# TravisWheelerLab/BATH

Hardware: AMD Instinct MI355X
Metric: DP Gcells/s + residues/s through bathsearch pipeline at 1/2/4/8 MI355X (higher is better)
Workload: dtype u8/i16 integer scores (SSV: exact binary16), f32 Forward

## Files before the change

### bath_amd/csrc/bath_orfs.hip

```cpp
#include <algorithm>
#include <climits>
#include <cstring>

#include "bath_common.hpp"
#include "bath_kernels.hpp"
#include "bath_launch.hpp"

namespace bath {

constexpr int kTileLanes = 32;
constexpr int kTileCodons = 4 * kTileLanes;
constexpr int kTileNt = 12 * kTileLanes;

struct OrfScanTables {
  const uint8_t *aa_full;
  const uint8_t *aa64_fwd;
  const uint8_t *aa64_rev;
  const uint8_t *comp;
};

struct OrfTiles {
  const int4 *desc;
  const int32_t *tile_first;
  int64_t ntiles;
};

struct OrfScanOut {
  uint8_t *aa;
  uint2 *slots;
  int32_t *cnt;
  uint2 *cross;
  int32_t *prefix, *suffix;
  int *hist;
  unsigned long long *n_orfs, *orf_res;
  int cap;
  int count;
};

struct OrfFilter {
  int strands;
  int using_initiators;
  const uint8_t *is_init;
  const uint8_t *comp;
};

__device__ __forceinline__ int orf_bin(int len) { return min(len, kOrfBins - 1); }

__device__ __forceinline__ int half_shfl_up(int v, int d) { return __shfl_up(v, d, kTileLanes); }

template <int CTRL, int ROW_MASK = 0xf>
__device__ __forceinline__ int dpp_or_ident(int v, int ident) { return __builtin_amdgcn_update_dpp(ident, v, CTRL, ROW_MASK, 0xf, false); }
__device__ __forceinline__ int half_excl_max_scan(int v, int ident, bool first_lane_of_half) {
  int x = dpp_or_ident<0x138>(v, ident);
  x = first_lane_of_half ? ident : x;
  x = max(x, dpp_or_ident<0x111>(x, ident));
  x = max(x, dpp_or_ident<0x112>(x, ident));
  x = max(x, dpp_or_ident<0x114>(x, ident));
  x = max(x, dpp_or_ident<0x118>(x, ident));
  x = max(x, dpp_or_ident<0x142, 0xa>(x, ident));
  return x;
}

__global__ __launch_bounds__(256) void orf_tile_kernel(SeqView dna, OrfTiles tiles, OrfScanTables tabs, OrfScanOut out, int minlen) {
  __shared__ int s_hist[kOrfBins];
  __shared__ __attribute__((aligned(16))) uint8_t s_full[5832 + 8];
  __shared__ uint16_t s_fr[64];
  __shared__ uint8_t s_comp[32];
  __shared__ unsigned s_red[2];
  __shared__ int s_cnt[8];
  for (int i = threadIdx.x; i < kOrfBins; i += blockDim.x) s_hist[i] = 0;
  for (int i = threadIdx.x; i < 5832; i += blockDim.x) s_full[i] = tabs.aa_full[i];
  if (threadIdx.x < 64) {
    const unsigned f = tabs.aa64_fwd[threadIdx.x], r = tabs.aa64_rev[threadIdx.x];
    s_fr[threadIdx.x] = (uint16_t)((f | (f == kStop ? 0x80u : 0u)) | ((r | (r == kStop ? 0x80u : 0u)) << 8));
  }
  if (threadIdx.x < 18) s_comp[threadIdx.x] = tabs.comp[threadIdx.x];
  if (threadIdx.x < 2) s_red[threadIdx.x] = 0;
  __syncthreads();
  const int hw = threadIdx.x / kTileLanes;
  const int i = threadIdx.x % kTileLanes;
  const int64_t wave0 = ((int64_t)blockIdx.x * blockDim.x + threadIdx.x) >> 6;
  const int64_t nwaves = ((int64_t)gridDim.x * blockDim.x) >> 6;
  unsigned my_orfs = 0, my_res = 0;
  const int half = (threadIdx.x & 63) / kTileLanes;
  const int4 none = {0, 0, 0, 0};
  auto fetch_desc = [&](int64_t tb) { const int64_t t = tb + half; return t < tiles.ntiles ? tiles.desc[t] : none; };
  auto fetch_data = [&](const int4 &dsc, uint32_t (&D)[4]) {
    const int p0 = kTileNt * dsc.w + 12 * i;
    D[0] = D[1] = D[2] = D[3] = 0u;
    if (p0 < dsc.y) {
      const uint8_t *d = dna.data + ((int64_t)(uint32_t)dsc.x << 4) + p0;
#pragma unroll
      for (int k = 0; k < 4; k++) D[k] = *reinterpret_cast<const uint32_t *>(d + 4 * k);
    }
  };
  const int64_t tstep = nwaves * 2;
  int4 d_next = fetch_desc(wave0 * 2), d_next2 = fetch_desc(wave0 * 2 + tstep);
  uint32_t D_next[4];
  fetch_data(d_next, D_next);
  for (int64_t tb = wave0 * 2; tb < tiles.ntiles; tb += tstep) {
    const int64_t tile = tb + half;
    const int4 dsc = d_next;
    uint32_t D[4] = {D_next[0], D_next[1], D_next[2], D_next[3]};
    d_next = d_next2;
    d_next2 = fetch_desc(tb + 2 * tstep);
    fetch_data(d_next, D_next);
    const int n = dsc.y;
    const bool live = n > 0;
    const int w = dsc.z, T = dsc.w;
    const int64_t off = (int64_t)(uint32_t)dsc.x << 4;
    const int p0 = kTileNt * T + 12 * i;
    if (i == 0) s_cnt[hw] = 0;
#pragma unroll
    for (int k = 0; k < 4; k++) {
      const int rem = n - (p0 + 4 * k);
      if (rem < 4) D[k] = (rem <= 0) ? 0u : (D[k] & ((1u << (8 * rem)) - 1u));
    }
    const bool canonical = ((D[0] | D[1] | D[2] | (D[3] & 0xffffu)) & 0xfcfcfcfcu) == 0u;
    int af[12], ar[12];
    if (__all(canonical)) {
#pragma unroll
      for (int k = 0; k < 12; k++) {
        const unsigned t = (k % 4 == 0) ? D[k / 4] : __builtin_amdgcn_alignbyte(D[k / 4 + 1], D[k / 4], k % 4);
        const unsigned idx = (__umul24(t, 0x100401u) >> 16) & 63u;
        const unsigned e = s_fr[idx];
        af[k] = (int)(e & 0xffu); ar[k] = (int)(e >> 8);
      }
    } else {
#pragma unroll
      for (int k = 0; k < 12; k++) {
        const unsigned t = (k % 4 == 0) ? D[k / 4] : __builtin_amdgcn_alignbyte(D[k / 4 + 1], D[k / 4], k % 4);
        const int x0 = min((int)(t & 0xffu), 17), x1 = min((int)((t >> 8) & 0xffu), 17), x2 = min((int)((t >> 16) & 0xffu), 17);
        const int f = s_full[(x0 * 18 + x1) * 18 + x2];
        const int r = s_full[((int)s_comp[x2] * 18 + (int)s_comp[x1]) * 18 + (int)s_comp[x0]];
        af[k] = f | (f == kStop ? 0x80 : 0); ar[k] = r | (r == kStop ? 0x80 : 0);
      }
    }
    const int nvalid = live ? min(max(n - 2 - p0, 0), 12) : 0;
    const int pitch = orf_stream_pitch(n);
    uint8_t *const abase = out.aa + (2 * off + 96 * (int64_t)w);
    const int u0 = kTileCodons * T + 4 * i;
    unsigned inv[3];
    int cv[3];
#pragma unroll
    for (int ph = 0; ph < 3; ph++) {
      cv[ph] = (max(nvalid - ph + 2, 0) * 11) >> 5;
      inv[ph] = cv[ph] >= 4 ? 0u : (0x80808080u << (8 * cv[ph]));
    }
    const int q3 = n / 3, r3 = n - 3 * q3;
    uint2 *const slots = out.slots + tile * out.cap;
    int *const prefix6 = out.prefix + tile * 6, *const suffix6 = out.suffix + tile * 6;
#pragma unroll
    for (int st = 0; st < 6; st++) {
      const int ph = st % 3;
      const bool rev = st >= 3;
      const int fr = r3 - ph + (r3 < ph ? 3 : 0);
      const int sf = rev ? 3 + fr : ph;
      const int C = q3 - 1 - (r3 < ph ? 1 : 0);
      const int *a = rev ? ar : af;
      const unsigned pk = (unsigned)a[ph] | ((unsigned)a[ph + 3] << 8) | ((unsigned)a[ph + 6] << 16) | ((unsigned)a[ph + 9] << 24);
      const unsigned mf = (pk & 0x80808080u) | inv[ph];
      const int so = sf * pitch + (rev ? C - u0 - 3 : u0);
      if (cv[ph] == 4) {
        *reinterpret_cast<uint32_t *>(abase + so) = rev ? __builtin_amdgcn_perm(0u, pk & 0x7f7f7f7fu, 0x00010203u)  : (pk & 0x7f7f7f7fu);
      } else {
#pragma unroll
        for (int c = 0; c < 4; c++) if (c < cv[ph]) abase[so + (rev ? 3 - c : c)] = (uint8_t)(a[ph + 3 * c] & 0x7f);
      }
      const int mine = mf ? 4 * i + ((31 - (int)__clz(mf)) >> 3) : INT_MIN;
      const int last = half_excl_max_scan(mine, INT_MIN, i == 0);
      bool open = last < 0;
      const int run_in = open ? 4 * i : 4 * i - 1 - last;
      auto record = [&](int u_stop, int len) {
        const int k = atomicAdd(&s_cnt[hw], 1);
        slots[k] = make_uint2((unsigned)(rev ? C - u_stop + 1 : u_stop - len), (unsigned)len | ((unsigned)sf << 28));
        atomicAdd(&s_hist[orf_bin(len)], 1);
        my_orfs++; my_res += (unsigned)len;
      };
      if (minlen > 2) {
        if (mf != 0u) {
          const int first = (__ffs((int)mf) - 1) >> 3;
          const int len = run_in + first;
          if (open) { if (live) prefix6[sf] = len; }
          else if (live && len >= minlen) record(u0 + first, len);
        }
        if (live && i == kTileLanes - 1) {
          suffix6[sf] = mf ? (int)__clz(mf) >> 3 : run_in + 4;
          if (open && mf == 0u) prefix6[sf] = kTileCodons;
        }
      } else {
        int len = run_in;
#pragma unroll
        for (int c = 0; c < 4; c++) {
          if ((mf >> (8 * c + 7)) & 1u) {
            if (open) { if (live) prefix6[sf] = len; open = false; }
            else if (live && len >= minlen) record(u0 + c, len);
            len = 0;
          } else len++;
        }
        if (live && i == kTileLanes - 1) {
          suffix6[sf] = len;
          if (open) prefix6[sf] = kTileCodons;
        }
      }
    }
    if (live && i == 0) out.cnt[tile] = s_cnt[hw];
  }
  if (my_orfs) { atomicAdd(&s_red[0], my_orfs); atomicAdd(&s_red[1], my_res); }
  __syncthreads();
  if (!out.count) return;
  for (int k = threadIdx.x; k < kOrfBins; k += blockDim.x) if (s_hist[k]) atomicAdd(&out.hist[k], s_hist[k]);
  if (threadIdx.x == 0 && s_red[0]) { atomicAdd(out.n_orfs, (unsigned long long)s_red[0]); atomicAdd(out.orf_res, (unsigned long long)s_red[1]); }
}

__global__ __launch_bounds__(256) void orf_stitch_kernel(SeqView dna, OrfTiles tiles, OrfScanOut out, int minlen) {
  __shared__ int s_hist[kOrfBins];
  __shared__ unsigned s_red[2];
  for (int i = threadIdx.x; i < kOrfBins; i += blockDim.x) s_hist[i] = 0;
  if (threadIdx.x < 2) s_red[threadIdx.x] = 0;
  __syncthreads();
  unsigned my_orfs = 0, my_res = 0;
  const int64_t nstreams = dna.n * 6;
  for (int64_t sidx = (int64_t)blockIdx.x * blockDim.x + threadIdx.x; sidx < nstreams; sidx += (int64_t)gridDim.x * blockDim.x) {
    const int64_t w = sidx / 6;
    const int sf = (int)(sidx - w * 6);
    const int n = dna.len[w];
    if (n < 15) continue;
    const int nt = (n / 3) / kTileCodons + 1;
    const int64_t first = tiles.tile_first[w];
    const bool rev = sf >= 3;
    const int fr = rev ? sf - 3 : 0;
    const int ph = rev ? (n - fr) % 3 : sf;
    const int C = (n - 3 - fr - ph) / 3;
    int carry = 0;
    for (int T = 0; T < nt; T++) {
      const int64_t e = (first + T) * 6 + sf;
      const int p = out.prefix[e];
      if (p < kTileCodons) {
        const int len = carry + p;
        uint2 none = make_uint2(0u, 0u);
        if (len < minlen) out.cross[e] = none;
        else {
          const int u_stop = kTileCodons * T + p;
          out.cross[e] = make_uint2((unsigned)(rev ? C - u_stop + 1 : u_stop - len), (unsigned)len | ((unsigned)sf << 28));
          atomicAdd(&s_hist[orf_bin(len)], 1);
          my_orfs++; my_res += (unsigned)len;
        }
        carry = out.suffix[e];
      } else { carry += kTileCodons; out.cross[e] = make_uint2(0u, 0u); }
    }
  }
  if (my_orfs) { atomicAdd(&s_red[0], my_orfs); atomicAdd(&s_red[1], my_res); }
  __syncthreads();
  if (!out.count) return;
  for (int k = threadIdx.x; k < kOrfBins; k += blockDim.x) if (s_hist[k]) atomicAdd(&out.hist[k], s_hist[k]);
  if (threadIdx.x == 0 && s_red[0]) { atomicAdd(out.n_orfs, (unsigned long long)s_red[0]); atomicAdd(out.orf_res, (unsigned long long)s_red[1]); }
}

__device__ __forceinline__ int wave_excl_max_scan(int v, int ident) {
  int x = dpp_or_ident<0x138>(v, ident);
  x = max(x, dpp_or_ident<0x111>(x, ident));
  x = max(x, dpp_or_ident<0x112>(x, ident));
  x = max(x, dpp_or_ident<0x114>(x, ident));
  x = max(x, dpp_or_ident<0x118>(x, ident));
  x = max(x, dpp_or_ident<0x142, 0xa>(x, ident));
  x = max(x, dpp_or_ident<0x143, 0xc>(x, ident));
  return x;
}
__global__ __launch_bounds__(256) void orf_stitch_wave_kernel(SeqView dna, OrfTiles tiles, OrfScanOut out, int minlen) {
  __shared__ int s_hist[kOrfBins];
  __shared__ unsigned s_red[2];
  for (int i = threadIdx.x; i < kOrfBins; i += blockDim.x) s_hist[i] = 0;
  if (threadIdx.x < 2) s_red[threadIdx.x] = 0;
  __syncthreads();
  unsigned my_orfs = 0, my_res = 0;
  const int lane = threadIdx.x & 63;
  const int64_t nstreams = dna.n * 6;
  const int64_t nwaves = ((int64_t)gridDim.x * blockDim.x) >> 6;
  for (int64_t sidx = ((int64_t)blockIdx.x * blockDim.x + threadIdx.x) >> 6; sidx < nstreams; sidx += nwaves) {
    const int64_t w = sidx / 6;
    const int sf = (int)(sidx - w * 6);
    const int n = dna.len[w];
    if (n < 15) continue;
    const int nt = (n / 3) / kTileCodons + 1;
    const int64_t first = tiles.tile_first[w];
    const bool rev = sf >= 3;
    const int fr = rev ? sf - 3 : 0;
    const int ph = rev ? (n - fr) % 3 : sf;
    const int C = (n - 3 - fr - ph) / 3;
    int carry_in = 0;
    for (int T0 = 0; T0 < nt; T0 += 64) {
      const int T = T0 + lane;
      const bool valid = T < nt;
      const int64_t e = (first + (valid ? T : 0)) * 6 + sf;
      const int p = valid ? out.prefix[e] : kTileCodons;
      const bool has = p < kTileCodons;
      const int sfx = has ? out.suffix[e] : 0;
      const int j = wave_excl_max_scan(has ? lane : -1, -1);
      const int sfx_j = __shfl(sfx, j < 0 ? 0 : j, 64);
      const int carry = (j >= 0) ? sfx_j + kTileCodons * (lane - j - 1) : carry_in + kTileCodons * lane;
      if (valid) {
        uint2 rec = make_uint2(0u, 0u);
        if (has) {
          const int len = carry + p;
          if (len >= minlen) {
            const int u_stop = kTileCodons * T + p;
            rec = make_uint2((unsigned)(rev ? C - u_stop + 1 : u_stop - len), (unsigned)len | ((unsigned)sf << 28));
            atomicAdd(&s_hist[orf_bin(len)], 1);
            my_orfs++; my_res += (unsigned)len;
          }
        }
        out.cross[e] = rec;
      }
      const int leave = has ? sfx : carry + kTileCodons;
      carry_in = __shfl(leave, 63, 64);
    }
  }
  if (my_orfs) { atomicAdd(&s_red[0], my_orfs); atomicAdd(&s_red[1], my_res); }
  __syncthreads();
  if (!out.count) return;
  for (int k = threadIdx.x; k < kOrfBins; k += blockDim.x) if (s_hist[k]) atomicAdd(&out.hist[k], s_hist[k]);
  if (threadIdx.x == 0 && s_red[0]) { atomicAdd(out.n_orfs, (unsigned long long)s_red[0]); atomicAdd(out.orf_res, (unsigned long long)s_red[1]); }
}

__global__ __launch_bounds__(256) void orf_filter_kernel(SeqView dna, OrfTiles tiles, OrfScanOut out, OrfFilter flt, int minlen) {
  __shared__ int s_hist[kOrfBins];
  __shared__ unsigned s_red[2];
  __shared__ uint8_t s_init[64], s_comp[32];
  for (int i = threadIdx.x; i < kOrfBins; i += blockDim.x) s_hist[i] = 0;
  if (threadIdx.x < 64) s_init[threadIdx.x] = flt.using_initiators ? flt.is_init[threadIdx.x] : 1;
  if (threadIdx.x < 18) s_comp[threadIdx.x] = flt.comp[threadIdx.x];
  if (threadIdx.x < 2) s_red[threadIdx.x] = 0;
  __syncthreads();
  auto members = [](int x) -> unsigned {
    switch (x) {
      case 0: return 1u; case 1: return 2u; case 2: return 4u; case 3: return 8u;
      case 5: return 5u; case 6: return 10u; case 7: return 3u; case 8: return 12u; case 9: return 6u; case 10: return 9u;
      case 11: return 11u; case 12: return 14u; case 13: return 7u; case 14: return 13u; case 15: return 15u;
      default: return 0u;
    }
  };
  auto initiates = [&](int a, int b, int c) -> bool {
    if ((a | b | c) < 4) return s_init[16 * a + 4 * b + c] != 0;
    const unsigned ma = members(a), mb = members(b), mc = members(c);
    int n = 0;
    for (int x = 0; x < 4; x++) if (ma >> x & 1u)
      for (int y = 0; y < 4; y++) if (mb >> y & 1u)
        for (int z = 0; z < 4; z++) if (mc >> z & 1u) { if (!s_init[16 * x + 4 * y + z]) return false; n++; }
    return n > 0;
  };
  unsigned my_orfs = 0, my_res = 0;
  for (int64_t t = (int64_t)blockIdx.x * blockDim.x + threadIdx.x; t < tiles.ntiles; t += (int64_t)gridDim.x * blockDim.x) {
    const int4 dsc = tiles.desc[t];
    const int n = dsc.y, w = dsc.z;
    if (n < 15) continue;
    const int64_t off = (int64_t)(uint32_t)dsc.x << 4;
    const uint8_t *x = dna.data + off;
    uint8_t *const abase = out.aa + (2 * off + 96 * (int64_t)w);
    const int pitch = orf_stream_pitch(n);
    const int c = out.cnt[t];
    uint2 *sl = out.slots + t * out.cap;
    for (int k = 0; k < c + 6; k++) {
      uint2 *rp = k < c ? sl + k : out.cross + t * 6 + (k - c);
      uint2 r = *rp;
      int len = (int)(r.y & 0x0fffffffu);
      if (len == 0) continue;
      const int sf = (int)(r.y >> 28);
      const bool rev = sf >= 3;
      if ((flt.strands == BATH_STRAND_TOPONLY && rev) || (flt.strands == BATH_STRAND_BOTTOMONLY && !rev)) { rp->y = 0u; continue; }
      if (flt.using_initiators) {
        int j = (int)r.x;
        const int jend = j + len;
        for (; j < jend; j++) {
          int a, b, cc;
          if (!rev) { const int p = sf + 3 * j; a = x[p]; b = x[p + 1]; cc = x[p + 2]; }
          else { const int q = (sf - 3) + 3 * j; a = s_comp[min((int)x[n - 1 - q], 17)]; b = s_comp[min((int)x[n - 2 - q], 17)]; cc = s_comp[min((int)x[n - 3 - q], 17)]; }
          if (initiates(min(a, 17), min(b, 17), min(cc, 17))) break;
        }
        len = jend - j;
        if (len < minlen || len <= 0) { rp->y = 0u; continue; }
        abase[sf * pitch + j] = 10;
        r.x = (unsigned)j; r.y = (unsigned)len | ((unsigned)sf << 28);
        *rp = r;
      }
      atomicAdd(&s_hist[orf_bin(len)], 1);
      my_orfs++; my_res += (unsigned)len;
    }
  }
  if (my_orfs) { atomicAdd(&s_red[0], my_orfs); atomicAdd(&s_red[1], my_res); }
  __syncthreads();
  for (int k = threadIdx.x; k < kOrfBins; k += blockDim.x) if (s_hist[k]) atomicAdd(&out.hist[k], s_hist[k]);
  if (threadIdx.x == 0 && s_red[0]) { atomicAdd(out.n_orfs, (unsigned long long)s_red[0]); atomicAdd(out.orf_res, (unsigned long long)s_red[1]); }
}

__global__ __launch_bounds__(256) void orf_scan_bins(const int *__restrict__ hist, int *__restrict__ cursor, int *__restrict__ n_total) {
  constexpr int kPer = kOrfBins / 256;
  __shared__ int s_wsum[4];
  const int tid = threadIdx.x, lane = tid & 63, wv = tid >> 6;
  int c[kPer], sum = 0;
#pragma unroll
  for (int k = 0; k < kPer; k++) { c[k] = hist[kOrfBins - 1 - (kPer * tid + k)]; sum += c[k]; }
  int x = sum;
#pragma unroll
  for (int d = 1; d < 64; d <<= 1) { const int y = __shfl_up(x, d, 64); if (lane >= d) x += y; }
  if (lane == 63) s_wsum[wv] = x;
  __syncthreads();
  int run = x - sum;
#pragma unroll
  for (int u = 0; u < 4; u++) run += u < wv ? s_wsum[u] : 0;
#pragma unroll
  for (int k = 0; k < kPer; k++) { cursor[(kOrfBins - 1 - (kPer * tid + k)) * kOrfCursorStride] = run; run += c[k]; }
  if (tid == 255) *n_total = run;
}

constexpr int kSortThreads = 1024;
constexpr int kSortTiles = 768;
constexpr int kSortRegs = 16;
constexpr int kSortRound = kSortThreads * kSortRegs;

__global__ __launch_bounds__(kSortThreads) void orf_sort_kernel(OrfTiles tiles, const uint2 *__restrict__ slots, int cap, const int32_t *__restrict__ cnt,
                                                                const uint2 *__restrict__ cross, int *__restrict__ cursor, OrfRec *__restrict__ sorted) {
  __shared__ int s_bin[kOrfBins];
  __shared__ int s_pre[kSortTiles + 1];
  __shared__ int64_t s_wbase[kSortTiles];
  __shared__ int2 s_wp[kSortTiles];
  __shared__ uint16_t s_own[kSortRound];
  __shared__ int s_wsum[kSortThreads / 64];
  const int tid = threadIdx.x, lane = tid & 63, wv = tid >> 6;
  const int64_t t0 = (int64_t)blockIdx.x * kSortTiles;
  int e = 0;
  if (tid < kSortTiles && t0 + tid < tiles.ntiles) {
    const int64_t t = t0 + tid;
    const int4 dsc = tiles.desc[t];
    e = cnt[t] + 6;
    s_wbase[tid] = 2 * ((int64_t)(uint32_t)dsc.x << 4) + 96 * (int64_t)dsc.z;
    s_wp[tid] = make_int2(dsc.z, orf_stream_pitch(dsc.y));
  }
  for (int i = tid; i < kOrfBins; i += kSortThreads) s_bin[i] = 0;
  int x = e;
#pragma unroll
  for (int d = 1; d < 64; d <<= 1) { const int y = __shfl_up(x, d, 64); if (lane >= d) x += y; }
  if (lane == 63) s_wsum[wv] = x;
  __syncthreads();
  int before = 0, total = 0;
#pragma unroll
  for (int u = 0; u < kSortThreads / 64; u++) { const int s = s_wsum[u]; before += u < wv ? s : 0; total += s; }
  const int pre = before + x - e;
  if (tid < kSortTiles) s_pre[tid] = pre;
  if (tid == 0) s_pre[kSortTiles] = total;
  for (int r0 = 0; r0 < total; r0 += kSortRound) {
    if (tid < kSortTiles) {
      const int lo = max(pre, r0) - r0, hi = min(pre + e, r0 + kSortRound) - r0;
      for (int j = lo; j < hi; j++) s_own[j] = (uint16_t)tid;
    }
    __syncthreads();
    uint2 r[kSortRegs];
    int ti[kSortRegs];
#pragma unroll
    for (int k = 0; k < kSortRegs; k++) {
      const int j = r0 + k * kSortThreads + tid;
      r[k] = make_uint2(0u, 0u);
      ti[k] = -1;
      if (j < total) {
        const int i = s_own[j - r0];
        const int loc = j - s_pre[i], c = s_pre[i + 1] - s_pre[i] - 6;
        const int64_t t = t0 + i;
        r[k] = loc < c ? slots[t * cap + loc] : cross[t * 6 + (loc - c)];
        ti[k] = i;
      }
    }
#pragma unroll
    for (int k = 0; k < kSortRegs; k++) {
      const int len = (int)(r[k].y & 0x0fffffffu);
      if (len) ti[k] |= atomicAdd(&s_bin[orf_bin(len)], 1) << 10;
      else ti[k] = -1;
    }
    __syncthreads();
    for (int i = tid; i < kOrfBins; i += kSortThreads) {
      const int c = s_bin[i];
      if (c) s_bin[i] = atomicAdd(&cursor[i * kOrfCursorStride], c);
    }
    __syncthreads();
#pragma unroll
    for (int k = 0; k < kSortRegs; k++) {
      if (ti[k] < 0) continue;
      const int i = ti[k] & 1023, rank = ti[k] >> 10;
      const int2 wp = s_wp[i];
      const int pos = s_bin[orf_bin((int)(r[k].y & 0x0fffffffu))] + rank;
      OrfRec rec;
      rec.aa_off = s_wbase[i] + (int64_t)(r[k].y >> 28) * wp.y + (int64_t)r[k].x; rec.w = wp.x; rec.len_sf = (int32_t)r[k].y;
      sorted[pos] = rec;
    }
    if (r0 + kSortRound < total) {
      __syncthreads();
      for (int i = tid; i < kOrfBins; i += kSortThreads) s_bin[i] = 0;
    }
  }
}

size_t orf_aa_bytes(const bath_hip_seqs *dna) { return (size_t)(2 * dna->total_aligned + 96 * dna->n + 256); }
void orf_buffers_carve(OrfBuffers *ob, void *aa, void *slots, void *sorted, void *misc, size_t nent) {
  ob->aa = static_cast<uint8_t *>(aa); ob->slots = slots; ob->sorted = static_cast<OrfRec *>(sorted);
  ob->cross = misc;
  ob->cnt = static_cast<int32_t *>(misc) + 2 * nent; ob->prefix = ob->cnt + nent; ob->suffix = ob->prefix + nent;
  ob->hist = reinterpret_cast<int *>(ob->suffix + nent); ob->cursor = ob->hist + kOrfBins; ob->ntotal = ob->cursor + kOrfBins * kOrfCursorStride;
}

int orf_slot_cap(int minlen) { return 6 * (kTileCodons / (std::max(minlen, 0) + 1) + 2); }

int orf_tiles_ensure(bath_hip_ctx *ctx, const bath_hip_seqs *dna) {
  if (dna->ntiles >= 0) return BATH_OK;
  std::vector<int32_t> first((size_t)std::max<int64_t>(dna->n, 1));
  std::vector<int4> desc;
  int64_t nt = 0;
  for (int64_t w = 0; w < dna->n; w++) {
    first[(size_t)w] = (int32_t)nt;
    const int n = dna->h_len[(size_t)w];
    const int k = n >= 15 ? (n / 3) / kTileCodons + 1 : 0;
    nt += k;
    if (nt >= (int64_t)INT32_MAX / 8 || (dna->h_off[(size_t)w] >> 4) > (int64_t)UINT32_MAX) { ctx->set_error("DNA block too large for one pipeline call: split it"); return BATH_EINVAL; }
    for (int T = 0; T < k; T++) desc.push_back(int4{(int)(uint32_t)(dna->h_off[(size_t)w] >> 4), n, (int)w, T});
  }
  if (desc.empty()) desc.push_back(int4{0, 0, 0, 0});
  BATH_HIP_TRY(ctx, hipMalloc((void **)&dna->d_tile_desc, desc.size() * sizeof(int4)));
  BATH_HIP_TRY(ctx, hipMalloc((void **)&dna->d_tile_first, first.size() * sizeof(int32_t)));
  BATH_HIP_TRY(ctx, hipMemcpy(dna->d_tile_desc, desc.data(), desc.size() * sizeof(int4), hipMemcpyHostToDevice));
  BATH_HIP_TRY(ctx, hipMemcpy(dna->d_tile_first, first.data(), first.size() * sizeof(int32_t), hipMemcpyHostToDevice));
  dna->ntiles = nt;
  return BATH_OK;
}

static bool dna_degen_has(int x, int y) {
  static const char *members[18] = {"A", "C", "G", "T", "", "AG", "CT", "AC", "GT", "CG", "AT", "ACT", "CGT", "ACG", "AGT", "ACGT", "", ""};
  static const char nt[] = "ACGT";
  return std::strchr(members[x], nt[y]) != nullptr;
}

static void build_codon_table(const uint8_t basic[64], std::vector<uint8_t> &tab) {
  tab.assign(18 * 18 * 18, (uint8_t)kXaa);
  for (int a = 0; a < 18; a++) for (int b = 0; b < 18; b++) for (int c = 0; c < 18; c++) {
    int aa = -1; bool mixed = false;
    for (int x = 0; x < 4 && !mixed; x++) { if (!dna_degen_has(a, x)) continue;
      for (int y = 0; y < 4 && !mixed; y++) { if (!dna_degen_has(b, y)) continue;
        for (int z = 0; z < 4; z++) { if (!dna_degen_has(c, z)) continue;
          int v = basic[16 * x + 4 * y + z];
          if (aa == -1) aa = v; else if (aa != v) { mixed = true; break; }
        } } }
    tab[(a * 18 + b) * 18 + c] = (uint8_t)((mixed || aa == -1) ? kXaa : aa);
  }
}

int orf_tables_upload(bath_hip_ctx *ctx, int ncbi_table, OrfTablesDev *t, int initiator) {
  const int key = ncbi_table | (initiator << 16);
  t->using_initiators = initiator != BATH_INIT_ANY;
  if (ctx->orf_tables_id == key && ctx->scratch[28].p) {
    t->full = ctx->scratch[28].as<uint8_t>(); t->fwd = t->full + 6144; t->rev = t->fwd + 64; t->comp = t->rev + 64; t->is_init = t->comp + 32;
    return BATH_OK;
  }
  uint8_t basic[64];
  if (bath_gencode_basic(ncbi_table, basic) != BATH_OK) { ctx->set_error("unknown NCBI translation table"); return BATH_EINVAL; }
  std::vector<uint8_t> host(6144 + 256, 0);
  std::vector<uint8_t> full;
  build_codon_table(basic, full);
  std::memcpy(host.data(), full.data(), full.size());
  uint8_t *fwd = host.data() + 6144, *rev = fwd + 64, *comp = rev + 64;
  for (int a = 0; a < 4; a++) for (int b = 0; b < 4; b++) for (int c = 0; c < 4; c++) {
    fwd[a * 16 + b * 4 + c] = basic[16 * a + 4 * b + c];
    rev[a * 16 + b * 4 + c] = basic[16 * (3 - c) + 4 * (3 - b) + (3 - a)];
  }
  static const uint8_t kComp[18] = {3, 2, 1, 0, 4, 6, 5, 8, 7, 9, 10, 14, 13, 12, 11, 15, 16, 17};
  std::memcpy(comp, kComp, 18);
  if (bath_gencode_initiators(ncbi_table, initiator, comp + 32) != BATH_OK) { ctx->set_error("no initiation codons for this table / initiator mode"); return BATH_EINVAL; }
  DevBuf &b = ctx->scratch[28];
  BATH_HIP_TRY(ctx, b.reserve(host.size()));
  BATH_HIP_TRY(ctx, hipMemcpyAsync(b.p, host.data(), host.size(), hipMemcpyHostToDevice, ctx->stream));
  BATH_HIP_TRY(ctx, hipStreamSynchronize(ctx->stream));
  ctx->orf_tables_id = key;
  t->full = b.as<uint8_t>(); t->fwd = t->full + 6144; t->rev = t->fwd + 64; t->comp = t->rev + 64; t->is_init = t->comp + 32;
  return BATH_OK;
}

int launch_orf_scan(bath_hip_ctx *ctx, const bath_hip_seqs *dna, const OrfTablesDev &tt, int minlen, const OrfBuffers &b,
                    unsigned long long *d_n_orfs, unsigned long long *d_orf_res, int strands) {
  const int64_t ntiles = dna->ntiles;
  BATH_HIP_TRY(ctx, hipMemsetAsync(b.hist, 0, kOrfBins * sizeof(int), ctx->stream));
  OrfScanTables tabs{tt.full, tt.fwd, tt.rev, tt.comp};
  OrfTiles tiles{reinterpret_cast<const int4 *>(dna->d_tile_desc), dna->d_tile_first, ntiles};
  const bool filtered = strands != BATH_STRAND_BOTH || tt.using_initiators;
  OrfScanOut out{b.aa, reinterpret_cast<uint2 *>(b.slots), b.cnt, reinterpret_cast<uint2 *>(b.cross), b.prefix, b.suffix, b.hist, d_n_orfs, d_orf_res, orf_slot_cap(minlen), filtered ? 0 : 1};
  const int cus = ctx->prop.multiProcessorCount;
  int per_cu = 0;
  if (hipOccupancyMaxActiveBlocksPerMultiprocessor(&per_cu, orf_tile_kernel, 256, 0) != hipSuccess || per_cu < 1) per_cu = 4;
  const int blocks = (int)std::max<int64_t>(1, std::min<int64_t>((ntiles + 7) / 8, (int64_t)cus * per_cu));
  hipLaunchKernelGGL(orf_tile_kernel, dim3(blocks), dim3(256), 0, ctx->stream, dna->view(), tiles, tabs, out, minlen);
  static const int stitch_env = [] { const char *e = std::getenv("BATH_HIP_STITCH_WAVE"); return e ? std::atoi(e) : -1; }();
  const bool long_windows = stitch_env >= 0 ? stitch_env == 1 : ntiles > 32 * dna->n;
  if (long_windows) {
    const int wblocks = (int)std::max<int64_t>(1, std::min<int64_t>((dna->n * 6 + 3) / 4, (int64_t)cus * 8));
    hipLaunchKernelGGL(orf_stitch_wave_kernel, dim3(wblocks), dim3(256), 0, ctx->stream, dna->view(), tiles, out, minlen);
  } else {
  const int sblocks = (int)std::max<int64_t>(1, std::min<int64_t>((dna->n * 6 + 255) / 256, (int64_t)cus * 8));
  hipLaunchKernelGGL(orf_stitch_kernel, dim3(sblocks), dim3(256), 0, ctx->stream, dna->view(), tiles, out, minlen);
  }
  if (filtered) {
    OrfFilter flt{strands, tt.using_initiators ? 1 : 0, tt.is_init, tt.comp};
    const int fblocks = (int)std::max<int64_t>(1, std::min<int64_t>((ntiles + 255) / 256, (int64_t)cus * 8));
    hipLaunchKernelGGL(orf_filter_kernel, dim3(fblocks), dim3(256), 0, ctx->stream, dna->view(), tiles, out, flt, minlen);
  }
  hipLaunchKernelGGL(orf_scan_bins, dim3(1), dim3(256), 0, ctx->stream, b.hist, b.cursor, b.ntotal);
  hipLaunchKernelGGL(orf_sort_kernel, dim3((unsigned)std::max<int64_t>(1, (ntiles + kSortTiles - 1) / kSortTiles)), dim3(kSortThreads), 0, ctx->stream, tiles,
                     reinterpret_cast<const uint2 *>(b.slots), out.cap, b.cnt, reinterpret_cast<const uint2 *>(b.cross), b.cursor, b.sorted);
  BATH_HIP_TRY(ctx, hipGetLastError());
  return BATH_OK;
}

}

using namespace bath;

extern "C" int bath_hip_translate_orfs(bath_hip_ctx *ctx, const bath_hip_seqs *dna, int ncbi_table, int min_orf_len,
                                       const bath_orf **orfs, int64_t *n_orfs, const uint8_t **aa) {
  return bath_hip_translate_orfs_opts(ctx, dna, ncbi_table, min_orf_len, BATH_STRAND_BOTH, BATH_INIT_ANY, orfs, n_orfs, aa);
}

extern "C" int bath_hip_translate_orfs_opts(bath_hip_ctx *ctx, const bath_hip_seqs *dna, int ncbi_table, int min_orf_len, int strands, int initiator,
                                            const bath_orf **orfs, int64_t *n_orfs, const uint8_t **aa) {
  if (!ctx || !dna || !orfs || !n_orfs || min_orf_len < 0 || strands < 0 || strands > 2 || initiator < 0 || initiator > 2) return BATH_EINVAL;
  BATH_HIP_TRY(ctx, hipSetDevice(ctx->device));
  *orfs = nullptr; *n_orfs = 0;
  if (aa) *aa = nullptr;
  ctx->orfs.clear(); ctx->orf_aa.clear(); ctx->orf_work.clear();
  if (dna->n == 0) return BATH_OK;
  int st;
  OrfTablesDev tt{};
  if ((st = orf_tables_upload(ctx, ncbi_table, &tt, initiator)) != BATH_OK) return st;
  if ((st = orf_tiles_ensure(ctx, dna)) != BATH_OK) return st;
  int64_t max_orfs = 0;
  for (int64_t i = 0; i < dna->n; i++) if (dna->h_len[i] >= 15) max_orfs += 6 * (int64_t)((dna->h_len[i] / 3 + 1) / (min_orf_len + 1) + 1);
  const size_t nent = (size_t)dna->ntiles * 6;
  DevBuf &b_aa = ctx->scratch[24], &b_slots = ctx->scratch[25], &b_orfs = ctx->scratch[26], &b_misc = ctx->scratch[27];
  BATH_HIP_TRY(ctx, b_aa.reserve(orf_aa_bytes(dna)));
  BATH_HIP_TRY(ctx, b_slots.reserve(((size_t)dna->ntiles * (size_t)orf_slot_cap(min_orf_len) + 64) * 8));
  BATH_HIP_TRY(ctx, b_orfs.reserve((size_t)(max_orfs + 64) * sizeof(OrfRec)));
  BATH_HIP_TRY(ctx, b_misc.reserve((5 * nent + kOrfMiscInts) * sizeof(int32_t) + 64));
  OrfBuffers ob{};
  orf_buffers_carve(&ob, b_aa.p, b_slots.p, b_orfs.p, b_misc.p, nent);
  unsigned long long *d_ctr = reinterpret_cast<unsigned long long *>(ob.ntotal + 2);
  BATH_HIP_TRY(ctx, hipMemsetAsync(d_ctr, 0, 16, ctx->stream));
  if ((st = launch_orf_scan(ctx, dna, tt, min_orf_len, ob, d_ctr, d_ctr + 1, strands)) != BATH_OK) return st;
  int total = 0;
  BATH_HIP_TRY(ctx, hipMemcpyAsync(&total, ob.ntotal, sizeof(int), hipMemcpyDeviceToHost, ctx->stream));
  BATH_HIP_TRY(ctx, hipStreamSynchronize(ctx->stream));
  std::vector<OrfRec> recs((size_t)total);
  std::vector<uint8_t> pool(orf_aa_bytes(dna));
  if (total > 0) BATH_HIP_TRY(ctx, hipMemcpy(recs.data(), ob.sorted, recs.size() * sizeof(OrfRec), hipMemcpyDeviceToHost));
  static_assert(sizeof(OrfRec) == sizeof(bath_orf_work), "bath_orf_work mirrors OrfRec");
  ctx->orf_work.resize((size_t)total);
  if (total > 0) std::memcpy(ctx->orf_work.data(), recs.data(), recs.size() * sizeof(OrfRec));
  BATH_HIP_TRY(ctx, hipMemcpy(pool.data(), ob.aa, pool.size(), hipMemcpyDeviceToHost));
  ctx->orfs.resize((size_t)total);
  for (int i = 0; i < total; i++) {
    const OrfRec &r = recs[(size_t)i];
    const int64_t w = r.w;
    const int sf = (int)((unsigned)r.len_sf >> 28), len = r.len_sf & 0x0fffffff;
    const int64_t stream = 2 * dna->h_off[w] + 96 * w + (int64_t)sf * orf_stream_pitch(dna->h_len[w]);
    bath_orf &o = ctx->orfs[(size_t)i];
    o.window = w; o.strand = sf / 3; o.frame = sf % 3; o.n = len;
    o.start = o.frame + 3 * (int32_t)(r.aa_off - stream) + 1; o.end = o.start + 3 * len - 1;
    o.aa_off = r.aa_off;
  }
  std::sort(ctx->orfs.begin(), ctx->orfs.end(), [](const bath_orf &a, const bath_orf &b) {
    if (a.window != b.window) return a.window < b.window;
    if (a.strand != b.strand) return a.strand < b.strand;
    if (a.frame != b.frame) return a.frame < b.frame;
    return a.start < b.start;
  });
  for (bath_orf &o : ctx->orfs) {
    const int64_t src = o.aa_off;
    o.aa_off = (int64_t)ctx->orf_aa.size();
    ctx->orf_aa.insert(ctx->orf_aa.end(), pool.begin() + src, pool.begin() + src + o.n);
  }
  *orfs = ctx->orfs.data(); *n_orfs = total;
  if (aa) *aa = ctx->orf_aa.data();
  return BATH_OK;
}

extern "C" int bath_hip_orf_worklist(bath_hip_ctx *ctx, const bath_orf_work **list, int64_t *n) {
  if (!ctx || !list || !n) return BATH_EINVAL;
  *list = ctx->orf_work.data(); *n = (int64_t)ctx->orf_work.size();
  return BATH_OK;
}
```

Measured before the change: 200.1 billion.

## Process eight codons per lane with 16-lane tiles in ORF tile kernel

Restructures the ORF tile scan so each lane handles 24 nucleotides (8 codons) instead of 12, with 16-lane tiles that fit within a DPP row, allowing a cheaper row-local max scan. Codon lookups are packed into 16-bit entries and permuted into 64-bit stop masks. Per-tile prefix/suffix/count values are staged in shared memory and written out cooperatively. It also adds an occupancy hint to launch bounds. The risks are higher register pressure from the wider per-lane state and changed tile geometry that must match the tile descriptors produced elsewhere.

```diff
diff --git a/bath_amd/csrc/bath_orfs.hip b/bath_amd/csrc/bath_orfs.hip
--- a/bath_amd/csrc/bath_orfs.hip
+++ b/bath_amd/csrc/bath_orfs.hip
@@ -8,9 +8,11 @@
 
 namespace bath {
 
-constexpr int kTileLanes = 32;
-constexpr int kTileCodons = 4 * kTileLanes;
-constexpr int kTileNt = 12 * kTileLanes;
+constexpr int kTileLanes = 16;
+constexpr int kLaneCodons = 8;
+constexpr int kLaneNt = 3 * kLaneCodons;
+constexpr int kTileCodons = kLaneCodons * kTileLanes;
+constexpr int kTileNt = kLaneNt * kTileLanes;
 
 struct OrfScanTables {
   const uint8_t *aa_full;
@@ -46,28 +48,24 @@
 
 __device__ __forceinline__ int orf_bin(int len) { return min(len, kOrfBins - 1); }
 
-__device__ __forceinline__ int half_shfl_up(int v, int d) { return __shfl_up(v, d, kTileLanes); }
-
 template <int CTRL, int ROW_MASK = 0xf>
 __device__ __forceinline__ int dpp_or_ident(int v, int ident) { return __builtin_amdgcn_update_dpp(ident, v, CTRL, ROW_MASK, 0xf, false); }
-__device__ __forceinline__ int half_excl_max_scan(int v, int ident, bool first_lane_of_half) {
-  int x = dpp_or_ident<0x138>(v, ident);
-  x = first_lane_of_half ? ident : x;
+__device__ __forceinline__ int row_excl_max_scan(int v, int ident) {
+  int x = dpp_or_ident<0x111>(v, ident);
   x = max(x, dpp_or_ident<0x111>(x, ident));
   x = max(x, dpp_or_ident<0x112>(x, ident));
   x = max(x, dpp_or_ident<0x114>(x, ident));
   x = max(x, dpp_or_ident<0x118>(x, ident));
-  x = max(x, dpp_or_ident<0x142, 0xa>(x, ident));
   return x;
 }
 
-__global__ __launch_bounds__(256) void orf_tile_kernel(SeqView dna, OrfTiles tiles, OrfScanTables tabs, OrfScanOut out, int minlen) {
+__global__ __launch_bounds__(256, 5) void orf_tile_kernel(SeqView dna, OrfTiles tiles, OrfScanTables tabs, OrfScanOut out, int minlen) {
   __shared__ int s_hist[kOrfBins];
   __shared__ __attribute__((aligned(16))) uint8_t s_full[5832 + 8];
   __shared__ uint16_t s_fr[64];
   __shared__ uint8_t s_comp[32];
   __shared__ unsigned s_red[2];
-  __shared__ int s_cnt[8];
+  __shared__ int s_sum[256 / kTileLanes][16];
   for (int i = threadIdx.x; i < kOrfBins; i += blockDim.x) s_hist[i] = 0;
   for (int i = threadIdx.x; i < 5832; i += blockDim.x) s_full[i] = tabs.aa_full[i];
   if (threadIdx.x < 64) {
@@ -77,31 +75,34 @@
   if (threadIdx.x < 18) s_comp[threadIdx.x] = tabs.comp[threadIdx.x];
   if (threadIdx.x < 2) s_red[threadIdx.x] = 0;
   __syncthreads();
-  const int hw = threadIdx.x / kTileLanes;
+  const int qw = threadIdx.x / kTileLanes;
   const int i = threadIdx.x % kTileLanes;
   const int64_t wave0 = ((int64_t)blockIdx.x * blockDim.x + threadIdx.x) >> 6;
   const int64_t nwaves = ((int64_t)gridDim.x * blockDim.x) >> 6;
   unsigned my_orfs = 0, my_res = 0;
-  const int half = (threadIdx.x & 63) / kTileLanes;
+  const int quarter = (threadIdx.x & 63) / kTileLanes;
   const int4 none = {0, 0, 0, 0};
-  auto fetch_desc = [&](int64_t tb) { const int64_t t = tb + half; return t < tiles.ntiles ? tiles.desc[t] : none; };
-  auto fetch_data = [&](const int4 &dsc, uint32_t (&D)[4]) {
-    const int p0 = kTileNt * dsc.w + 12 * i;
-    D[0] = D[1] = D[2] = D[3] = 0u;
-    if (p0 < dsc.y) {
-      const uint8_t *d = dna.data + ((int64_t)(uint32_t)dsc.x << 4) + p0;
-#pragma unroll
-      for (int k = 0; k < 4; k++) D[k] = *reinterpret_cast<const uint32_t *>(d + 4 * k);
-    }
+  auto fetch_desc = [&](int64_t tb) { const int64_t t = tb + quarter; return t < tiles.ntiles ? tiles.desc[t] : none; };
+  auto fetch_data = [&](const int4 &dsc, uint32_t (&D)[7]) {
+    const int p0 = kTileNt * dsc.w + kLaneNt * i;
+#pragma unroll
+    for (int k = 0; k < 7; k++) D[k] = 0u;
+    const uint8_t *d = dna.data + ((int64_t)(uint32_t)dsc.x << 4) + p0;
+#pragma unroll
+    for (int k = 0; k < 3; k++)
+      if (p0 + 8 * k < dsc.y) { const uint2 v = *reinterpret_cast<const uint2 *>(d + 8 * k); D[2 * k] = v.x; D[2 * k + 1] = v.y; }
+    if (p0 + 24 < dsc.y) D[6] = *reinterpret_cast<const uint32_t *>(d + 24);
   };
-  const int64_t tstep = nwaves * 2;
-  int4 d_next = fetch_desc(wave0 * 2), d_next2 = fetch_desc(wave0 * 2 + tstep);
-  uint32_t D_next[4];
+  const int64_t tstep = nwaves * 4;
+  int4 d_next = fetch_desc(wave0 * 4), d_next2 = fetch_desc(wave0 * 4 + tstep);
+  uint32_t D_next[7];
   fetch_data(d_next, D_next);
-  for (int64_t tb = wave0 * 2; tb < tiles.ntiles; tb += tstep) {
-    const int64_t tile = tb + half;
+  for (int64_t tb = wave0 * 4; tb < tiles.ntiles; tb += tstep) {
+    const int64_t tile = tb + quarter;
     const int4 dsc = d_next;
-    uint32_t D[4] = {D_next[0], D_next[1], D_next[2], D_next[3]};
+    uint32_t D[7];
+#pragma unroll
+    for (int k = 0; k < 7; k++) D[k] = D_next[k];
     d_next = d_next2;
     d_next2 = fetch_desc(tb + 2 * tstep);
     fetch_data(d_next, D_next);
@@ -109,47 +110,54 @@
     const bool live = n > 0;
     const int w = dsc.z, T = dsc.w;
     const int64_t off = (int64_t)(uint32_t)dsc.x << 4;
-    const int p0 = kTileNt * T + 12 * i;
-    if (i == 0) s_cnt[hw] = 0;
-#pragma unroll
-    for (int k = 0; k < 4; k++) {
-      const int rem = n - (p0 + 4 * k);
-      if (rem < 4) D[k] = (rem <= 0) ? 0u : (D[k] & ((1u << (8 * rem)) - 1u));
-    }
-    const bool canonical = ((D[0] | D[1] | D[2] | (D[3] & 0xffffu)) & 0xfcfcfcfcu) == 0u;
-    int af[12], ar[12];
+    const int p0 = kTileNt * T + kLaneNt * i;
+    if (i == 0) s_sum[qw][12] = 0;
+    const int rem8 = 8 * min(n - p0, 32);
+#pragma unroll
+    for (int k = 0; k < 7; k++) {
+      const int t8 = min(max(rem8 - 32 * k, 0), 32);
+      D[k] &= (uint32_t)((0xffffffffull << t8) >> 32);
+    }
+    const bool canonical = ((D[0] | D[1] | D[2] | D[3] | D[4] | D[5] | (D[6] & 0xffffu)) & 0xfcfcfcfcu) == 0u;
+    unsigned W[12];
     if (__all(canonical)) {
-#pragma unroll
-      for (int k = 0; k < 12; k++) {
+      unsigned e[24];
+#pragma unroll
+      for (int k = 0; k < 24; k++) {
         const unsigned t = (k % 4 == 0) ? D[k / 4] : __builtin_amdgcn_alignbyte(D[k / 4 + 1], D[k / 4], k % 4);
-        const unsigned idx = (__umul24(t, 0x100401u) >> 16) & 63u;
-        const unsigned e = s_fr[idx];
-        af[k] = (int)(e & 0xffu); ar[k] = (int)(e >> 8);
+        const unsigned boff = (__umul24(t, 0x200802u) >> 16) & 127u;
+        e[k] = *reinterpret_cast<const uint16_t *>(reinterpret_cast<const uint8_t *>(s_fr) + boff);
       }
+#pragma unroll
+      for (int q = 0; q < 12; q++) W[q] = e[q / 4 + 6 * (q % 4)] | (e[q / 4 + 6 * (q % 4) + 3] << 16);
     } else {
-#pragma unroll
-      for (int k = 0; k < 12; k++) {
+      unsigned e[24];
+#pragma unroll
+      for (int k = 0; k < 24; k++) {
         const unsigned t = (k % 4 == 0) ? D[k / 4] : __builtin_amdgcn_alignbyte(D[k / 4 + 1], D[k / 4], k % 4);
         const int x0 = min((int)(t & 0xffu), 17), x1 = min((int)((t >> 8) & 0xffu), 17), x2 = min((int)((t >> 16) & 0xffu), 17);
-        const int f = s_full[(x0 * 18 + x1) * 18 + x2];
-        const int r = s_full[((int)s_comp[x2] * 18 + (int)s_comp[x1]) * 18 + (int)s_comp[x0]];
-        af[k] = f | (f == kStop ? 0x80 : 0); ar[k] = r | (r == kStop ? 0x80 : 0);
+        const unsigned f = s_full[(x0 * 18 + x1) * 18 + x2];
+        const unsigned r = s_full[((int)s_comp[x2] * 18 + (int)s_comp[x1]) * 18 + (int)s_comp[x0]];
+        e[k] = (f | (f == kStop ? 0x80u : 0u)) | ((r | (r == kStop ? 0x80u : 0u)) << 8);
       }
-    }
-    const int nvalid = live ? min(max(n - 2 - p0, 0), 12) : 0;
+#pragma unroll
+      for (int q = 0; q < 12; q++) W[q] = e[q / 4 + 6 * (q % 4)] | (e[q / 4 + 6 * (q % 4) + 3] << 16);
+    }
+    const int nvalid = live ? min(max(n - 2 - p0, 0), kLaneNt) : 0;
     const int pitch = orf_stream_pitch(n);
     uint8_t *const abase = out.aa + (2 * off + 96 * (int64_t)w);
-    const int u0 = kTileCodons * T + 4 * i;
-    unsigned inv[3];
+    const int u0 = kTileCodons * T + kLaneCodons * i;
+    unsigned long long inv_f[3], inv_r[3];
     int cv[3];
 #pragma unroll
     for (int ph = 0; ph < 3; ph++) {
-      cv[ph] = (max(nvalid - ph + 2, 0) * 11) >> 5;
-      inv[ph] = cv[ph] >= 4 ? 0u : (0x80808080u << (8 * cv[ph]));
+      cv[ph] = ((nvalid - ph + 2) * 43) >> 7;
+      inv_f[ph] = cv[ph] >= kLaneCodons ? 0ull : (0x8080808080808080ull << (8 * cv[ph]));
+      inv_r[ph] = cv[ph] >= kLaneCodons ? 0ull : (0x8080808080808080ull >> (8 * cv[ph]));
     }
     const int q3 = n / 3, r3 = n - 3 * q3;
     uint2 *const slots = out.slots + tile * out.cap;
-    int *const prefix6 = out.prefix + tile * 6, *const suffix6 = out.suffix + tile * 6;
+    int *const prefix6 = &s_sum[qw][0], *const suffix6 = &s_sum[qw][6];
 #pragma unroll
     for (int st = 0; st < 6; st++) {
       const int ph = st % 3;
@@ -157,42 +165,52 @@
       const int fr = r3 - ph + (r3 < ph ? 3 : 0);
       const int sf = rev ? 3 + fr : ph;
       const int C = q3 - 1 - (r3 < ph ? 1 : 0);
-      const int *a = rev ? ar : af;
-      const unsigned pk = (unsigned)a[ph] | ((unsigned)a[ph + 3] << 8) | ((unsigned)a[ph + 6] << 16) | ((unsigned)a[ph + 9] << 24);
-      const unsigned mf = (pk & 0x80808080u) | inv[ph];
-      const int so = sf * pitch + (rev ? C - u0 - 3 : u0);
-      if (cv[ph] == 4) {
-        *reinterpret_cast<uint32_t *>(abase + so) = rev ? __builtin_amdgcn_perm(0u, pk & 0x7f7f7f7fu, 0x00010203u)  : (pk & 0x7f7f7f7fu);
-      } else {
-#pragma unroll
-        for (int c = 0; c < 4; c++) if (c < cv[ph]) abase[so + (rev ? 3 - c : c)] = (uint8_t)(a[ph + 3 * c] & 0x7f);
+      const unsigned lo = rev ? __builtin_amdgcn_perm(W[4 * ph + 3], W[4 * ph + 2], 0x01030507u) : __builtin_amdgcn_perm(W[4 * ph + 1], W[4 * ph + 0], 0x06040200u);
+      const unsigned hi = rev ? __builtin_amdgcn_perm(W[4 * ph + 1], W[4 * ph + 0], 0x01030507u) : __builtin_amdgcn_perm(W[4 * ph + 3], W[4 * ph + 2], 0x06040200u);
+      const unsigned long long mf = (((unsigned long long)(hi & 0x80808080u) << 32) | (unsigned long long)(lo & 0x80808080u)) | (rev ? inv_r[ph] : inv_f[ph]);
+      const int so = sf * pitch + (rev ? C - u0 - (kLaneCodons - 1) : u0);
+      uint8_t *const ap = abase + so;
+      const unsigned lo7 = lo & 0x7f7f7f7fu, hi7 = hi & 0x7f7f7f7fu;
+      if (cv[ph] == kLaneCodons) {
+        *reinterpret_cast<uint32_t *>(ap) = lo7;
+        *reinterpret_cast<uint32_t *>(ap + 4) = hi7;
+      } else if (cv[ph] > 0) {
+        unsigned long long v = ((unsigned long long)hi7 << 32) | lo7;
+        uint8_t *q = ap;
+        if (rev) { v >>= 8 * (kLaneCodons - cv[ph]); q += kLaneCodons - cv[ph]; }
+        if (cv[ph] & 4) { *reinterpret_cast<uint32_t *>(q) = (uint32_t)v; v >>= 32; q += 4; }
+        if (cv[ph] & 2) { *reinterpret_cast<uint16_t *>(q) = (uint16_t)v; v >>= 16; q += 2; }
+        if (cv[ph] & 1) *q = (uint8_t)v;
       }
-      const int mine = mf ? 4 * i + ((31 - (int)__clz(mf)) >> 3) : INT_MIN;
-      const int last = half_excl_max_scan(mine, INT_MIN, i == 0);
+      const bool any = mf != 0ull;
+      const int b_top = (63 - (int)__clzll((long long)mf)) >> 3, b_bot = (__ffsll((long long)mf) - 1) >> 3;
+      const int c_last = rev ? kLaneCodons - 1 - b_bot : b_top;
+      const int c_first = rev ? kLaneCodons - 1 - b_top : b_bot;
+      const int mine = any ? kLaneCodons * i + c_last : INT_MIN;
+      const int last = row_excl_max_scan(mine, INT_MIN);
       bool open = last < 0;
-      const int run_in = open ? 4 * i : 4 * i - 1 - last;
+      const int run_in = open ? kLaneCodons * i : kLaneCodons * i - 1 - last;
       auto record = [&](int u_stop, int len) {
-        const int k = atomicAdd(&s_cnt[hw], 1);
+        const int k = atomicAdd(&s_sum[qw][12], 1);
         slots[k] = make_uint2((unsigned)(rev ? C - u_stop + 1 : u_stop - len), (unsigned)len | ((unsigned)sf << 28));
         atomicAdd(&s_hist[orf_bin(len)], 1);
         my_orfs++; my_res += (unsigned)len;
       };
-      if (minlen > 2) {
-        if (mf != 0u) {
-          const int first = (__ffs((int)mf) - 1) >> 3;
-          const int len = run_in + first;
+      if (minlen > kLaneCodons - 2) {
+        if (any) {
+          const int len = run_in + c_first;
           if (open) { if (live) prefix6[sf] = len; }
-          else if (live && len >= minlen) record(u0 + first, len);
+          else if (live && len >= minlen) record(u0 + c_first, len);
         }
         if (live && i == kTileLanes - 1) {
-          suffix6[sf] = mf ? (int)__clz(mf) >> 3 : run_in + 4;
-          if (open && mf == 0u) prefix6[sf] = kTileCodons;
+          suffix6[sf] = any ? kLaneCodons - 1 - c_last : run_in + kLaneCodons;
+          if (open && !any) prefix6[sf] = kTileCodons;
         }
       } else {
         int len = run_in;
 #pragma unroll
-        for (int c = 0; c < 4; c++) {
-          if ((mf >> (8 * c + 7)) & 1u) {
+        for (int c = 0; c < kLaneCodons; c++) {
+          if ((mf >> (8 * (rev ? kLaneCodons - 1 - c : c) + 7)) & 1ull) {
             if (open) { if (live) prefix6[sf] = len; open = false; }
             else if (live && len >= minlen) record(u0 + c, len);
             len = 0;
@@ -204,7 +222,11 @@
         }
       }
     }
-    if (live && i == 0) out.cnt[tile] = s_cnt[hw];
+    __builtin_amdgcn_fence(__ATOMIC_ACQ_REL, "wavefront");
+    if (live && i < 13) {
+      int *const dst = i < 6 ? out.prefix + tile * 6 + i : i < 12 ? out.suffix + tile * 6 + (i - 6) : out.cnt + tile;
+      *dst = s_sum[qw][i];
+    }
   }
   if (my_orfs) { atomicAdd(&s_red[0], my_orfs); atomicAdd(&s_red[1], my_res); }
   __syncthreads();
@@ -591,7 +613,7 @@
   const int cus = ctx->prop.multiProcessorCount;
   int per_cu = 0;
   if (hipOccupancyMaxActiveBlocksPerMultiprocessor(&per_cu, orf_tile_kernel, 256, 0) != hipSuccess || per_cu < 1) per_cu = 4;
-  const int blocks = (int)std::max<int64_t>(1, std::min<int64_t>((ntiles + 7) / 8, (int64_t)cus * per_cu));
+  const int blocks = (int)std::max<int64_t>(1, std::min<int64_t>((ntiles + 15) / 16, (int64_t)cus * per_cu));
   hipLaunchKernelGGL(orf_tile_kernel, dim3(blocks), dim3(256), 0, ctx->stream, dna->view(), tiles, tabs, out, minlen);
   static const int stitch_env = [] { const char *e = std::getenv("BATH_HIP_STITCH_WAVE"); return e ? std::atoi(e) : -1; }();
   const bool long_windows = stitch_env >= 0 ? stitch_env == 1 : ntiles > 32 * dna->n;
```

Result: faster. 204.2 billion (median of 6 runs) (+2.1%).
